# rcedgar/muscle

Hardware: AMD Instinct MI355X
Metric: sequence-pairs/sec (fwd+bwd+posterior+relax) (higher is better)
Workload: dtype f32

## Files before the change

### muscle_amd/csrc/kernels_store.h

```cpp
#pragma once
#include "device_math.h"

struct __attribute__((aligned(8))) MpcEnt { u32 p; u32 c; };

struct StoreParams {
	u32 n;
	const u32 *seq_len;
	u64 npairs;
	const u32 *pair_x, *pair_y;
	u32 *packed;
	const u64 *pbase;
	const u64 *vbase;
	u32 *rp;
	const u64 *rp_base;
	MpcEnt *ent;
	const u64 *ent_base;
	const u32 *mbase;
	float *vnext;
	u32 *pad;
	u32 lcap1;
	unsigned short *pos_f, *pos_t;
	const u32 *rec_off;
	u32 *ovf_off;
	u32 nb1;
	u32 *win;
	const u32 *wrec_off;
	u32 *wv_off;
	unsigned short *pos_wf, *pos_wt;
	u32 nrect;
	const u32 *rects;
	const u8 *need;
	const u64 *pad_zbase, *win_zbase;
	const u32 *pad_zend, *win_zend;
};

#define MPC_PAD_ROW 2
#define MPC_WIN_MAXSPAN 31u
#define MPC_WIN_MAXOFF 32767u
#define MPC_RB_HB 8u
#define MPC_PAD_SENTINEL 0x1fffu

__device__ __forceinline__ u64 mpc_pair_index(u32 n, u32 i, u32 j)
{
	return (u64)i * n - ((u64)i * (i + 1)) / 2 + (j - i - 1);
}

__device__ __forceinline__ u64 mpc_pair_pos_f(u32 n, u32 nrect, const u32 *rects, u32 X, u32 Y)
{
	if (nrect == 0u) return mpc_pair_index(n, X, Y);
	for (u32 r = 0; r < nrect; ++r) {
		const u32 *q = rects + 6u * r;
		const u32 xa = q[0], xb = q[1], ya = q[2], yb = q[3];
		if (X < xa || X >= xb || Y < ya || Y >= yb) continue;
		const u64 base = (u64)q[4] | ((u64)q[5] << 32);
		return ya >= xb ? base + (u64)(X - xa) * (yb - ya) + (Y - ya) : base + mpc_pair_index(xb - xa, X - xa, Y - xa);
	}
	return ~0ull;
}
__device__ __forceinline__ u64 mpc_pair_pos(const StoreParams &s, u32 X, u32 Y) { return mpc_pair_pos_f(s.n, s.nrect, s.rects, X, Y); }
__device__ __forceinline__ bool mpc_need(const StoreParams &s, u32 A) { return s.need == nullptr || s.need[A] != 0; }

__device__ __forceinline__ u64 mpc_rec_index(u32 n, u32 A, u32 Z) { return (u64)Z * n + A; }
__device__ __forceinline__ u32 *mpc_rec_ptr(const StoreParams &s, u32 A, u32 Z)
{
	u32 *base = s.pad_zbase ? (u32 *)s.pad_zbase[Z] : s.pad;
	return base + 4 * (u64)s.rec_off[mpc_rec_index(s.n, A, Z)];
}
__device__ __forceinline__ u32 *mpc_wrec_ptr(const StoreParams &s, u32 A, u32 Z)
{
	u32 *base = s.win_zbase ? (u32 *)s.win_zbase[Z] : s.win;
	return base + 4 * (u64)s.wrec_off[mpc_rec_index(s.n, A, Z)];
}
__device__ __forceinline__ u32 mpc_rec_end(const StoreParams &s, u32 A, u32 Z) { return (s.pad_zend && A + 1u == s.n) ? s.pad_zend[Z] : s.rec_off[mpc_rec_index(s.n, A, Z) + 1]; }
__device__ __forceinline__ u32 mpc_wrec_end(const StoreParams &s, u32 A, u32 Z) { return (s.win_zend && A + 1u == s.n) ? s.win_zend[Z] : s.wrec_off[mpc_rec_index(s.n, A, Z) + 1]; }
__device__ __forceinline__ bool mpc_has_win(const StoreParams &s) { return s.win != nullptr || s.win_zbase != nullptr; }

__global__ void __launch_bounds__(64) slab_build_kernel(StoreParams s)
{
	const int t = threadIdx.x;
	const u64 total = (u64)s.n * s.n;
	for (u64 b = blockIdx.x; b < total; b += gridDim.x) {
		const u32 A = (u32)(b / s.n), Z = (u32)(b % s.n);
		const u32 LA = s.seq_len[A];
		u32 *rp = s.rp + s.rp_base[A] + (u64)Z * (LA + 1);
		const u32 mb = s.mbase[(u64)A * (s.n + 1) + Z];
		if (A == Z) {
			for (u32 a = t; a <= LA; a += 64) rp[a] = mb;
			continue;
		}
		const bool fwd = A < Z;
		const u64 k = fwd ? mpc_pair_pos(s, A, Z) : mpc_pair_pos(s, Z, A);
		const u32 *rec = s.packed + s.pbase[k];
		const u32 LX = fwd ? LA : s.seq_len[Z];
		const u32 LY = fwd ? s.seq_len[Z] : LA;
		const u32 nnz = (u32)(s.vbase[k + 1] - s.vbase[k]);
		const u32 *cnt = fwd ? rec : rec + LX;
		u32 carry = mb;
		for (u32 a0 = 0; a0 <= LA; a0 += 64) {
			const u32 a = a0 + t;
			const u32 v = (a < LA) ? cnt[a] : 0;
			u32 incl = v;
			for (int d = 1; d < 64; d <<= 1) {
				const u32 o = __shfl_up(incl, d);
				if (t >= d) incl += o;
			}
			if (a <= LA) rp[a] = carry + incl - v;
			carry += __shfl(incl, 63);
		}
		const u32 *e = rec + LX + LY;
		const u32 *rowv = e + 2 * (u64)nnz;
		const u32 *tperm = rowv + nnz;
		MpcEnt *dst = s.ent + s.ent_base[A] + mb;
		for (u32 q = t; q < nnz; q += 64) {
			MpcEnt v;
			v.p = e[2 * (u64)q];
			if (fwd) { v.c = e[2 * (u64)q + 1]; dst[q] = v; }
			else { v.c = rowv[q]; dst[tperm[q]] = v; }
		}
	}
}

__global__ void __launch_bounds__(64) var_size_kernel(StoreParams s, u32 *sizes)
{
	const int t = threadIdx.x;
	const u64 total = (u64)s.n * s.n;
	for (u64 b = blockIdx.x; b < total; b += gridDim.x) {
		const u32 Z = (u32)(b / s.n), A = (u32)(b % s.n);
		const u32 LA = s.seq_len[A];
		u32 mine = 0;
		if (!mpc_need(s, A)) { if (t == 0) sizes[b] = 0u; continue; }
		if (A != Z) {
			const bool fwd = A < Z;
			const u64 k = fwd ? mpc_pair_pos(s, A, Z) : mpc_pair_pos(s, Z, A);
			const u32 *rec = s.packed + s.pbase[k];
			const u32 *cnt = fwd ? rec : rec + s.seq_len[Z];
			for (u32 a = t; a < LA; a += 64) {
				const u32 nb = (cnt[a] + MPC_PAD_ROW - 1) / MPC_PAD_ROW;
				mine += nb > 1 ? nb - 1 : 0;
			}
			for (int d = 32; d >= 1; d >>= 1) mine += __shfl_down(mine, d);
		}
		if (t == 0) sizes[b] = LA + mine;
	}
}

__global__ void __launch_bounds__(64) var_build_kernel(StoreParams s)
{
	MPC_DYN_SMEM(smem_raw);
	u32 *s_start = (u32 *)smem_raw;
	u32 *s_ovf = s_start + s.lcap1;
	const int t = threadIdx.x;
	const u64 total = (u64)s.n * s.n;
	for (u64 b = blockIdx.x; b < total; b += gridDim.x) {
		const u32 Z = (u32)(b / s.n), A = (u32)(b % s.n);
		const u32 LA = s.seq_len[A];
		if (!mpc_need(s, A)) continue;
		u32 *rec_out = mpc_rec_ptr(s, A, Z);
		const u32 rec_end = mpc_rec_end(s, A, Z);
		const u32 units = rec_end - s.rec_off[b];
		for (u32 q = t; q < units; q += 64) {
			rec_out[4 * q] = 0u; rec_out[4 * q + 1] = 0u; rec_out[4 * q + 2] = MPC_PAD_SENTINEL; rec_out[4 * q + 3] = MPC_PAD_SENTINEL;
		}
		if (A == Z) {
			if (s.ovf_off) for (u32 q = t; q < s.nb1; q += 64) s.ovf_off[b * s.nb1 + q] = rec_end;
			continue;
		}
		const bool fwd = A < Z;
		const u64 k = fwd ? mpc_pair_pos(s, A, Z) : mpc_pair_pos(s, Z, A);
		const u32 *rec = s.packed + s.pbase[k];
		const u32 LX = fwd ? LA : s.seq_len[Z];
		const u32 LY = fwd ? s.seq_len[Z] : LA;
		const u32 nnz = (u32)(s.vbase[k + 1] - s.vbase[k]);
		const u32 *cnt = fwd ? rec : rec + LX;
		u32 carry = 0, carry_o = 0;
		for (u32 a0 = 0; a0 < LA; a0 += 64) {
			const u32 a = a0 + t;
			const u32 v = (a < LA) ? cnt[a] : 0;
			const u32 nb = (v + MPC_PAD_ROW - 1) / MPC_PAD_ROW;
			const u32 vo = nb > 1 ? nb - 1 : 0;
			u32 incl = v, incl_o = vo;
			for (int d = 1; d < 64; d <<= 1) {
				const u32 o = __shfl_up(incl, d), oo = __shfl_up(incl_o, d);
				if (t >= d) { incl += o; incl_o += oo; }
			}
			if (a < LA) {
				s_start[a] = carry + incl - v;
				s_ovf[a] = carry_o + incl_o - vo;
			}
			carry += __shfl(incl, 63);
			carry_o += __shfl(incl_o, 63);
		}
		__syncthreads();
		if (s.ovf_off)
			for (u32 q = t; q < s.nb1; q += 64)
				s.ovf_off[b * s.nb1 + q] = MPC_RB_HB * q < LA ? s.rec_off[b] + LA + s_ovf[MPC_RB_HB * q] : rec_end;
		const u32 *e = rec + LX + LY;
		const u32 *rowv = e + 2 * (u64)nnz;
		const u32 *tperm = rowv + nnz;
		unsigned short *pos = (fwd ? s.pos_f : s.pos_t) + s.vbase[k];
		for (u32 q = t; q < nnz; q += 64) {
			const u32 pbits = e[2 * (u64)q];
			const u32 col = e[2 * (u64)q + 1], row = rowv[q];
			const u32 r = fwd ? row : col;
			const u32 rank = fwd ? q : tperm[q];
			const u32 c = fwd ? col : row;
			const u32 within = rank - s_start[r];
			const u32 j = within / MPC_PAD_ROW, slot = within % MPC_PAD_ROW;
			const u32 nb = (cnt[r] + MPC_PAD_ROW - 1) / MPC_PAD_ROW;
			const u32 ovf0 = LA + s_ovf[r];
			const u32 unit = j == 0 ? r : ovf0 + (j - 1);
			const u32 delta = j + 1 < nb ? (j == 0 ? ovf0 - r : 1u) : 0u;
			rec_out[4 * unit + slot] = pbits;
			rec_out[4 * unit + 2 + slot] = slot == 0 ? (c | (delta << 20)) : c;
			if (slot == 0 && within + 1 == cnt[r]) rec_out[4 * unit + 3] = c;
			pos[q] = (unsigned short)(unit * MPC_PAD_ROW + slot);
		}
		__syncthreads();
	}
}

__global__ void __launch_bounds__(64) win_size_kernel(StoreParams s, u32 *sizes, u32 *vals_total, u32 *too_wide)
{
	const int t = threadIdx.x;
	const u64 total = (u64)s.n * s.n;
	for (u64 b = blockIdx.x; b < total; b += gridDim.x) {
		const u32 Z = (u32)(b / s.n), A = (u32)(b % s.n);
		const u32 LA = s.seq_len[A];
		u32 mine = 0;
		if (!mpc_need(s, A)) { if (t == 0) { sizes[b] = 0u; vals_total[b] = 0u; } continue; }
		if (A != Z) {
			const u32 *rec = mpc_rec_ptr(s, A, Z);
			for (u32 a = t; a < LA; a += 64) {
				u32 blk = a;
				const u32 c_first = rec[4 * blk + 2] & 0xffffu;
				u32 span = 0;
				if (c_first != MPC_PAD_SENTINEL) {
					for (u32 d = rec[4 * blk + 2] >> 20; d != 0u; d = rec[4 * blk + 2] >> 20) blk += d;
					span = rec[4 * blk + 3] - c_first + 1u;
				}
				mine += span + 1u;
			}
			for (int d = 32; d >= 1; d >>= 1) mine += __shfl_down(mine, d);
		} else mine = LA;
		if (t == 0) {
			sizes[b] = (LA + 1u + 3u) / 4u + (mine + 3u) / 4u + 1u;
			vals_total[b] = mine;
			if (mine > MPC_WIN_MAXOFF) atomicOr(too_wide, 1u);
		}
	}
}

__global__ void __launch_bounds__(64) win_build_kernel(StoreParams s)
{
	MPC_DYN_SMEM(smem_raw);
	u32 *s_off = (u32 *)smem_raw;
	const u32 t = threadIdx.x;
	const u64 total = (u64)s.n * s.n;
	for (u64 b = blockIdx.x; b < total; b += gridDim.x) {
		const u32 Z = (u32)(b / s.n), A = (u32)(b % s.n);
		const u32 LA = s.seq_len[A];
		if (!mpc_need(s, A)) continue;
		const u32 *rec = mpc_rec_ptr(s, A, Z);
		u32 *wrec = mpc_wrec_ptr(s, A, Z);
		const u32 dblocks = (LA + 1u + 3u) / 4u;
		u32 *desc = wrec, *vals = wrec + 4 * (u64)dblocks;
		u32 carry = 0;
		for (u32 a0 = 0; a0 <= LA; a0 += 64) {
			const u32 a = a0 + t;
			u32 c_first = 0, span = 0;
			if (a < LA) {
				u32 blk = a;
				const u32 cf = rec[4 * blk + 2] & 0xffffu;
				if (cf != MPC_PAD_SENTINEL) {
					for (u32 d = rec[4 * blk + 2] >> 20; d != 0u; d = rec[4 * blk + 2] >> 20) blk += d;
					c_first = cf; span = rec[4 * blk + 3] - cf + 1u;
				}
			}
			const u32 v = a < LA ? span + 1u : 0u;
			u32 incl = v;
			for (int d = 1; d < 64; d <<= 1) {
				const u32 o = __shfl_up(incl, d);
				if (t >= (u32)d) incl += o;
			}
			const u32 off = carry + incl - v;
			if (a <= LA) { desc[a] = c_first | ((span < MPC_WIN_MAXSPAN ? span : MPC_WIN_MAXSPAN) << 12) | (off << 17); s_off[a] = off; }
			carry += __shfl(incl, 63);
		}
		for (u32 q = LA + 1u + t; q < 4u * dblocks; q += 64) desc[q] = carry << 17;
		__syncthreads();
		const u32 vtotal = carry, vblocks = (vtotal + 3u) / 4u + 1u;
		for (u32 q = t; q < 4u * vblocks; q += 64) vals[q] = 0u;
		if (s.wv_off)
			for (u32 q = t; q < s.nb1; q += 64)
				s.wv_off[b * s.nb1 + q] = MPC_RB_HB * q < LA ? s.wrec_off[b] + dblocks + s_off[MPC_RB_HB * q] / 4u : mpc_wrec_end(s, A, Z) - 1u;
		__syncthreads();
		for (u32 a = t; a < LA; a += 64) {
			u32 blk = a;
			const u32 cf = rec[4 * blk + 2] & 0xffffu;
			if (cf == MPC_PAD_SENTINEL) continue;
			const u32 off = s_off[a];
			for (;;) {
				const u32 c0 = rec[4 * blk + 2] & 0xffffu, c1 = rec[4 * blk + 3];
				vals[off + (c0 - cf)] = rec[4 * blk];
				if (c1 != c0) vals[off + (c1 - cf)] = rec[4 * blk + 1];
				const u32 d = rec[4 * blk + 2] >> 20;
				if (d == 0u) break;
				blk += d;
			}
		}
		__syncthreads();
	}
}

__global__ void __launch_bounds__(64) win_pos_kernel(StoreParams s)
{
	const u32 t = threadIdx.x;
	for (u64 k = blockIdx.x; k < s.npairs; k += gridDim.x) {
		const u32 X = s.pair_x[k], Y = s.pair_y[k];
		const u32 LX = s.seq_len[X], LY = s.seq_len[Y];
		const u32 *prec = s.packed + s.pbase[k];
		const u32 *ent = prec + LX + LY;
		const u32 nnz = (u32)(s.vbase[k + 1] - s.vbase[k]);
		const bool nx = mpc_need(s, X), ny = mpc_need(s, Y);
		if (!nx && !ny) continue;
		const u32 *dxy = mpc_wrec_ptr(s, X, Y);
		const u32 *dyx = mpc_wrec_ptr(s, Y, X);
		for (u32 q = t; q < nnz; q += 64) {
			const u32 col = ent[2 * (u64)q + 1], row = ent[2 * (u64)nnz + q];
			if (nx) { const u32 wf = dxy[row]; s.pos_wf[s.vbase[k] + q] = (unsigned short)((wf >> 17) + (col - (wf & 0xfffu))); }
			if (ny) { const u32 wt = dyx[col]; s.pos_wt[s.vbase[k] + q] = (unsigned short)((wt >> 17) + (row - (wt & 0xfffu))); }
		}
	}
}

__device__ __forceinline__ void mpc_tile_runs(u32 x0, u32 nx, u32 y0, u32 ny, u32 *ys, u32 *nys)
{
	const u32 lo = y0 > x0 + nx ? y0 : x0 + nx, hi = y0 + ny;
	*ys = lo;
	*nys = hi > lo ? hi - lo : 0u;
}

__global__ void __launch_bounds__(64) var_tile_fit_kernel(StoreParams s, const u32 *tiles, u32 ntiles, u32 *out)
{
	const u32 t = threadIdx.x, n = s.n;
	for (u32 tl = blockIdx.x; tl < ntiles; tl += gridDim.x) {
		const u32 x0 = tiles[4 * tl], nx = tiles[4 * tl + 1], y0 = tiles[4 * tl + 2], ny = tiles[4 * tl + 3];
		u32 ys, nys;
		mpc_tile_runs(x0, nx, y0, ny, &ys, &nys);
		u32 best = 0;
		for (u32 Z = t; Z < n; Z += 64) {
			const u64 bx = mpc_rec_index(n, x0, Z);
			u32 sum = mpc_rec_end(s, x0 + nx - 1u, Z) - s.rec_off[bx];
			if (nys) { const u64 by = mpc_rec_index(n, ys, Z); sum += mpc_rec_end(s, ys + nys - 1u, Z) - s.rec_off[by]; }
			best = sum > best ? sum : best;
		}
		for (int d = 32; d >= 1; d >>= 1) { const u32 o = __shfl_down(best, d); best = o > best ? o : best; }
		if (t == 0) out[tl] = best;
	}
}

__device__ __forceinline__ u64 mpc_find_pair(const u64 *vbase, u64 lo, u64 hi, u64 e)
{
	while (hi - lo > 1) {
		const u64 mid = (lo + hi) >> 1;
		if (vbase[mid] <= e) lo = mid; else hi = mid;
	}
	return lo;
}

__global__ void __launch_bounds__(256) relax_kernel(StoreParams s, u64 k0, u64 k1)
{
	const u64 first = s.vbase[k0], last = s.vbase[k1];
	const u32 n = s.n;
	for (u64 e = first + (u64)blockIdx.x * blockDim.x + threadIdx.x; e < last; e += (u64)gridDim.x * blockDim.x) {
		const u64 k = mpc_find_pair(s.vbase, k0, k1, e);
		const u32 X = s.pair_x[k], Y = s.pair_y[k];
		const u32 LX = s.seq_len[X], LY = s.seq_len[Y];
		const u32 *rec = s.packed + s.pbase[k];
		const u32 nnz = (u32)(s.vbase[k + 1] - s.vbase[k]);
		const u32 idx = (u32)(e - s.vbase[k]);
		const u32 *ent = rec + LX + LY;
		const float pxy = __uint_as_float(ent[2 * (u64)idx]);
		const u32 y = ent[2 * (u64)idx + 1];
		const u32 x = ent[2 * (u64)nnz + idx];
		float acc = pxy * 2.0f;
		const u32 *rpx = s.rp + s.rp_base[X] + x;
		const u32 *rpy = s.rp + s.rp_base[Y] + y;
		const MpcEnt *ex = s.ent + s.ent_base[X];
		const MpcEnt *ey = s.ent + s.ent_base[Y];
		const u32 sxs = LX + 1, sys = LY + 1;
		for (u32 Z = 0; Z < n; ++Z) {
			u32 a = rpx[0], a1 = rpx[1];
			u32 b = rpy[0], b1 = rpy[1];
			rpx += sxs; rpy += sys;
			if (a == a1 || b == b1) continue;
			MpcEnt va = ex[a], vb = ey[b];
			for (;;) {
				if (va.c == vb.c) {
					acc += __uint_as_float(va.p) * __uint_as_float(vb.p);
					if (++a == a1 || ++b == b1) break;
					va = ex[a]; vb = ey[b];
				} else if (va.c < vb.c) {
					if (++a == a1) break;
					va = ex[a];
				} else {
					if (++b == b1) break;
					vb = ey[b];
				}
			}
		}
		s.vnext[e] = acc / (float)n;
	}
}

__global__ void __launch_bounds__(256) commit_kernel(StoreParams s, u64 e0, u64 e1)
{
	const u64 last = e1;
	for (u64 e = e0 + (u64)blockIdx.x * blockDim.x + threadIdx.x; e < last; e += (u64)gridDim.x * blockDim.x) {
		const u64 k = mpc_find_pair(s.vbase, 0, s.npairs, e);
		const u32 X = s.pair_x[k], Y = s.pair_y[k];
		const u32 LX = s.seq_len[X], LY = s.seq_len[Y];
		u32 *rec = s.packed + s.pbase[k];
		const u32 nnz = (u32)(s.vbase[k + 1] - s.vbase[k]);
		const u32 idx = (u32)(e - s.vbase[k]);
		u32 *ent = rec + LX + LY;
		const u32 pb = __float_as_uint(s.vnext[e]);
		const u32 tq = ent[3 * (u64)nnz + idx];
		ent[2 * (u64)idx] = pb;
		s.ent[s.ent_base[X] + s.mbase[(u64)X * (s.n + 1) + Y] + idx].p = pb;
		s.ent[s.ent_base[Y] + s.mbase[(u64)Y * (s.n + 1) + X] + tq].p = pb;
	}
}

__global__ void __launch_bounds__(64) commit_pairs_kernel(StoreParams s, u64 k0, u64 k1, u64 e0, u64 e1, u64 own0, u64 own1, int lazy_packed)
{
	const u32 t = threadIdx.x;
	for (u64 k = k0 + blockIdx.x; k < k1; k += gridDim.x) {
		const u32 X = s.pair_x[k], Y = s.pair_y[k];
		const bool nx = mpc_need(s, X), ny = mpc_need(s, Y);
		const bool pk = !lazy_packed || (k >= own0 && k < own1);
		if (!nx && !ny && !pk) continue;
		const u64 vb = s.vbase[k], ve = s.vbase[k + 1];
		const u64 a = vb > e0 ? vb : e0, b = ve < e1 ? ve : e1;
		if (a >= b) continue;
		const u32 LX = s.seq_len[X], LY = s.seq_len[Y];
		u32 *ent = s.packed + s.pbase[k] + LX + LY;
		u32 *rx = mpc_rec_ptr(s, X, Y), *ry = mpc_rec_ptr(s, Y, X);
		const bool hw = mpc_has_win(s);
		u32 *wx = hw ? mpc_wrec_ptr(s, X, Y) + 4 * (u64)((LX + 1u + 3u) / 4u) : nullptr;
		u32 *wy = hw ? mpc_wrec_ptr(s, Y, X) + 4 * (u64)((LY + 1u + 3u) / 4u) : nullptr;
		for (u64 e = a + t; e < b; e += 64) {
			const u32 pb = __float_as_uint(s.vnext[e]);
			if (pk) ent[2 * (e - vb)] = pb;
			if (nx) { const u32 pf = s.pos_f[e]; rx[(pf >> 1) * 4u + (pf & 1u)] = pb; if (wx) wx[s.pos_wf[e]] = pb; }
			if (ny) { const u32 pt = s.pos_t[e]; ry[(pt >> 1) * 4u + (pt & 1u)] = pb; if (wy) wy[s.pos_wt[e]] = pb; }
		}
	}
}

__global__ void __launch_bounds__(64) packed_refresh_kernel(StoreParams s, u64 k0, u64 k1, u64 e0, u64 e1, u64 own0, u64 own1)
{
	const u32 t = threadIdx.x;
	for (u64 k = k0 + blockIdx.x; k < k1; k += gridDim.x) {
		if (k >= own0 && k < own1) continue;
		const u64 vb = s.vbase[k], ve = s.vbase[k + 1];
		const u64 a = vb > e0 ? vb : e0, b = ve < e1 ? ve : e1;
		u32 *ent = s.packed + s.pbase[k] + s.seq_len[s.pair_x[k]] + s.seq_len[s.pair_y[k]];
		for (u64 e = a + t; e < b; e += 64) ent[2 * (e - vb)] = __float_as_uint(s.vnext[e]);
	}
}

__global__ void __launch_bounds__(256) pack_kernel(const u32 *res, u64 res_stride, const u64 *dst_base,
	const u64 *rec_words, u32 *packed, u32 count)
{
	for (u32 pid = blockIdx.x; pid < count; pid += gridDim.x) {
		const u32 *src = res + (u64)pid * res_stride;
		u32 *dst = packed + dst_base[pid];
		const u64 w = rec_words[pid];
		for (u64 q = threadIdx.x; q < w; q += blockDim.x) dst[q] = src[q];
	}
}

__global__ void __launch_bounds__(64) export_kernel(StoreParams s, u64 k0, u64 k1, const u64 *off_base,
	u32 *out_off, u32 *out_val, const u64 *klist, const u64 *val_base)
{
	const int t = threadIdx.x;
	for (u64 q = k0 + blockIdx.x; q < k1; q += gridDim.x) {
		const u64 k = klist ? klist[q] : q;
		const u32 LX = s.seq_len[s.pair_x[k]], LY = s.seq_len[s.pair_y[k]];
		const u32 *rec = s.packed + s.pbase[k];
		const u32 nnz = (u32)(s.vbase[k + 1] - s.vbase[k]);
		u32 *oo = out_off + off_base[q - k0];
		u32 carry = 0;
		for (u32 a0 = 0; a0 <= LX; a0 += 64) {
			const u32 a = a0 + t;
			const u32 v = (a < LX) ? rec[a] : 0;
			u32 incl = v;
			for (int d = 1; d < 64; d <<= 1) {
				const u32 o = __shfl_up(incl, d);
				if (t >= d) incl += o;
			}
			if (a <= LX) oo[a] = carry + incl - v;
			carry += __shfl(incl, 63);
		}
		const u32 *ent = rec + LX + LY;
		u32 *ov = out_val + 2 * (klist ? val_base[q] : s.vbase[k] - s.vbase[k0]);
		for (u32 i = t; i < 2 * nnz; i += 64) ov[i] = ent[i];
	}
}
```

### muscle_amd/csrc/mpcgpu_store.inc

```

const u64 kStoreSegBlocksMax = 0xffffffffull;

bool plan_store_segments(u32 n, const u32 *sizes, u64 limit, std::vector<u32> &z_first, std::vector<u64> &blocks)
{
	z_first.assign(1, 0u);
	blocks.assign(1, 0ull);
	for (u32 Z = 0; Z < n; ++Z) {
		u64 slab = 0;
		for (u32 A = 0; A < n; ++A) slab += sizes[(u64)Z * n + A];
		if (slab > limit) return false;
		if (blocks.back() + slab > limit) { z_first.push_back(Z); blocks.push_back(0ull); }
		blocks.back() += slab;
	}
	return true;
}

u64 store_seg_limit()
{
	const char *e = getenv("MPCGPU_STORE_SEG_BLOCKS");
	const u64 v = (e && *e) ? strtoull(e, nullptr, 10) : 0ull;
	return (v == 0ull || v > kStoreSegBlocksMax) ? kStoreSegBlocksMax : v;
}

void segment_offsets(u32 n, std::vector<u32> &off, const std::vector<u32> &z_first, std::vector<u32> &zend)
{
	zend.resize(n);
	u64 run = 0;
	size_t g = 0;
	for (u32 Z = 0; Z < n; ++Z) {
		if (g + 1 < z_first.size() && Z == z_first[g + 1]) { ++g; run = 0; }
		for (u32 A = 0; A < n; ++A) {
			const u64 b = (u64)Z * n + A;
			const u32 sz = off[b + 1];
			off[b] = (u32)run;
			run += sz;
		}
		zend[Z] = (u32)run;
	}
	off[(u64)n * n] = (u32)run;
}

bool segments_held(const DevBuf &one, const SegStore &st, const std::vector<u64> &blocks)
{
	if (blocks.size() == 1) return one.cap >= std::max<u64>(blocks[0], 1) * 16;
	if (st.seg.size() != blocks.size()) return false;
	for (size_t g = 0; g < blocks.size(); ++g)
		if (st.seg[g].cap < std::max<u64>(blocks[g], 1) * 16) return false;
	return true;
}

int alloc_segments(mpcgpu_ctx *c, SegStore &st, const std::vector<u32> &z_first, const std::vector<u64> &blocks, const std::vector<u32> &zend)
{
	const u32 n = c->n;
	for (size_t g = blocks.size(); g < st.seg.size(); ++g) st.seg[g].release();
	st.seg.resize(blocks.size());
	std::vector<u64> zb(n);
	for (size_t g = 0; g < blocks.size(); ++g) {
		HIPCHK(c, st.seg[g].ensure(std::max<u64>(blocks[g], 1) * 16));
		const u32 z1 = g + 1 < blocks.size() ? z_first[g + 1] : n;
		for (u32 Z = z_first[g]; Z < z1; ++Z) zb[Z] = (u64)(uintptr_t)st.seg[g].p;
	}
	if (upload(c, st.zbase, zb) || upload(c, st.zend, zend)) return 1;
	HIPCHK(c, hipStreamSynchronize(c->stream));
	return 0;
}

int build_var_store(mpcgpu_ctx *c)
{
	const u32 n = c->n;
	if (c->max_len > MPC_RV_MAXLEN) return 2;
	StoreParams sp0;
	fill_store_params(c, sp0);
	const u64 nn = (u64)n * n;
	HIPCHK(c, c->d_sizes.ensure(nn * 4));
	MPC_LAUNCH(var_size_kernel, (u32)std::min<u64>(nn, (u64)c->prop.multiProcessorCount * 32), 64, 0, c->stream, sp0, c->d_sizes.as<u32>());
	HIPCHK(c, hipGetLastError());
	std::vector<u32> &off = c->v_off;
	off.resize(nn + 1);
	HIPCHK(c, hipMemcpyAsync(off.data() + 1, c->d_sizes.p, nn * 4, hipMemcpyDeviceToHost, c->stream));
	HIPCHK(c, hipStreamSynchronize(c->stream));
	off[0] = 0;
	u32 max_rec = 0;
	u64 run = 0;
	for (u64 b = 0; b < nn; ++b) { max_rec = std::max(max_rec, off[b + 1]); run += off[b + 1]; }
	if (max_rec > 4095u) return 2;
	const u64 seg_limit = store_seg_limit();
	std::vector<u32> seg_z, zend;
	std::vector<u64> seg_blocks;
	if (!plan_store_segments(n, off.data() + 1, seg_limit, seg_z, seg_blocks)) return 2;
	const u32 nseg = (u32)seg_blocks.size();
	segment_offsets(n, off, seg_z, zend);
	auto fits = [&](bool fallback) {
		return 2ull * max_rec * 16 <= var_buf_bytes(fallback) && (((u64)c->max_nnz + 63) & ~63ull) <= (u64)var_max_slots(fallback) * 1024u;
	};
	const bool fits_primary = fits(false), pairs_ok = fits_primary || fits(true);
	const char *tiles_mode = getenv("MPCGPU_RELAX_TILES");
	const int small_n = env_int("MPCGPU_RELAX_SMALL_PAIRS", 0);
	const bool small_pairs = small_n > 0 && n <= (u32)small_n && fits_primary && !(tiles_mode && !strcmp(tiles_mode, "band")) && nseg == 1;
	const bool want_band = !(tiles_mode && !strcmp(tiles_mode, "pairs")) && !small_pairs && c->npairs < 0xffffffffull;
	if (nseg > 1 && tiles_mode && !strcmp(tiles_mode, "pairs"))
		return fail(c, "MPCGPU_RELAX_TILES=pairs: the whole-record tiles of relax_var_kernel do not read a record store in segments "
			"(%u segments of at most %llu blocks; band tiles do)", nseg, (u64)seg_limit);
	c->var_mixed = !fits_primary && pairs_ok;
	if (!pairs_ok && !want_band) return 2;
	if (nseg > 1 && !want_band) return 2;
	const u64 pad_bytes = run * 16 + 4 * std::max<u64>(c->total_entries, 1);
	const bool held = segments_held(c->d_pad, c->pad_seg, seg_blocks) && 4 * std::max<u64>(c->total_entries, 1) <= c->d_pos.cap;
	if (!segments_held(c->d_pad, c->pad_seg, seg_blocks)) { c->d_pad.release(); c->pad_seg.release(); }
	size_t freeb = 0, totb = 0;
	HIPCHK(c, hipMemGetInfo(&freeb, &totb));
	if (!(held || pad_bytes + ((u64)2 << 30) <= (u64)freeb)) return 2;
	c->d_rp.release(); c->d_ent.release(); c->d_mbase.release();
	if (nseg == 1) {
		c->pad_seg.release();
		HIPCHK(c, c->d_pad.ensure(std::max<u64>(run, 1) * 16));
	} else {
		c->d_pad.release();
		if (alloc_segments(c, c->pad_seg, seg_z, seg_blocks, zend)) return 1;
	}
	HIPCHK(c, c->d_pos.ensure(4 * std::max<u64>(c->total_entries, 1)));
	if (upload(c, c->d_rec_off, off)) return 1;
	HIPCHK(c, hipStreamSynchronize(c->stream));
	c->have_pad = true;
	c->pad_lcap1 = c->max_len;
	c->var_max_rec_blocks = max_rec; c->var_total_blocks = run;
	c->tiles_k0 = c->tiles_k1 = ~0ull;
	{
		char b[512];
		snprintf(b, sizeof(b), "variable-size dense records: %u x %u records, %.2f GB, mean %.0f B, largest %u B; relax_var_kernel, 2 x 1024-thread workgroups per CU, 1 staging buffer of %u B",
			n, n, (double)run * 16 / 1e9, (double)run * 16 / (double)nn, max_rec * 16, var_buf_bytes(false));
		c->store_desc = b;
		if (c->var_mixed) c->store_desc += " (pairs whose records do not fit it: 1 x 1024-thread workgroup per CU with 160 KB, second launch)";
		if (nseg > 1) c->store_desc += " in " + std::to_string(nseg) + " segments of whole Z slabs";
		c->tiles_desc.clear(); c->relax_kernel_name.clear(); c->relax_fallback = false;
	}
	c->band_ok = false;
	c->btiles_k0 = c->btiles_k1 = ~0ull;
	{
		const u32 nb1 = (c->max_len + MPC_RB_HB - 1) / MPC_RB_HB + 1;
		const u64 tab_bytes = (nn + 2 * c->npairs + 2ull * n) * nb1 * 4;
		size_t free2 = 0, tot2 = 0;
		HIPCHK(c, hipMemGetInfo(&free2, &tot2));
		if (want_band && (c->d_ovf_off.cap >= nn * nb1 * 4 || tab_bytes + ((u64)1 << 30) <= (u64)free2)) {
			HIPCHK(c, c->d_ovf_off.ensure(nn * nb1 * 4));
			HIPCHK(c, c->d_cell_off.ensure(std::max<u64>(c->npairs, 1) * nb1 * 4));
			HIPCHK(c, c->d_yr.ensure(std::max<u64>(c->npairs, 1) * nb1 * 4));
			HIPCHK(c, c->d_ovf_sum.ensure(3ull * n * nb1 * 4));
			HIPCHK(c, c->d_ovf_maxc.ensure((u64)n * nb1 * 4));
			c->band_ok = true;
			c->band_nb1 = nb1;
			char b[256];
			snprintf(b, sizeof(b), "variable-size dense records: %u x %u records, %.2f GB, mean %.0f B, largest %u B, band index of %u rows",
				n, n, (double)run * 16 / 1e9, (double)run * 16 / (double)nn, max_rec * 16, (unsigned)MPC_RB_HB);
			c->store_desc = b;
			if (nseg > 1) c->store_desc += ", in " + std::to_string(nseg) + " segments of whole Z slabs";
		}
		if (!c->band_ok && (!pairs_ok || nseg > 1)) { c->have_pad = false; return 2; }
		c->var_pairs_ok = pairs_ok && nseg == 1;
	}
	StoreParams sp;
	fill_store_params(c, sp);
	if (trace_on()) {
		fprintf(stderr, "[mpcgpu] store: variable-size dense records, %u x %u records, %.2f GB (mean %.0f B, largest %u B)%s\n", n, n,
			(double)run * 16 / 1e9, (double)run * 16 / (double)nn, max_rec * 16, c->var_mixed ? ", relax_var fallback for the largest pairs" : "");
		fflush(stderr);
	}
	TimedSpan ts;
	if (span_begin(c, 2, &ts)) return 1;
	MPC_LAUNCH(var_build_kernel, (u32)std::min<u64>(nn, (u64)c->prop.multiProcessorCount * 32), 64, (size_t)std::max(sp.lcap1, 1u) * 8, c->stream, sp);
	HIPCHK(c, hipGetLastError());
	c->win_ok = false;
	{
		const char *form = getenv("MPCGPU_RELAX_FORM");
		if (c->band_ok && !(form && !strcmp(form, "walk"))) {
			HIPCHK(c, c->d_sizes.ensure(nn * 4));
			HIPCHK(c, c->d_tilefit.ensure(nn * 4));
			HIPCHK(c, c->d_wflag.ensure(4));
			HIPCHK(c, hipMemsetAsync(c->d_wflag.p, 0, 4, c->stream));
			MPC_LAUNCH(win_size_kernel, (u32)std::min<u64>(nn, (u64)c->prop.multiProcessorCount * 32), 64, 0, c->stream, sp, c->d_sizes.as<u32>(),
				c->d_tilefit.as<u32>(), c->d_wflag.as<u32>());
			HIPCHK(c, hipGetLastError());
			std::vector<u32> &woff = c->v_woff;
			woff.resize(nn + 1);
			u32 wide = 0;
			HIPCHK(c, hipMemcpyAsync(woff.data() + 1, c->d_sizes.p, nn * 4, hipMemcpyDeviceToHost, c->stream));
			HIPCHK(c, hipMemcpyAsync(&wide, c->d_wflag.p, 4, hipMemcpyDeviceToHost, c->stream));
			HIPCHK(c, hipStreamSynchronize(c->stream));
			woff[0] = 0;
			u64 wrun = 0;
			for (u64 b = 0; b < nn; ++b) wrun += woff[b + 1];
			std::vector<u32> wseg_z, wzend;
			std::vector<u64> wseg_blocks;
			const bool wplan = plan_store_segments(n, woff.data() + 1, seg_limit, wseg_z, wseg_blocks);
			const u32 nwseg = wplan ? (u32)wseg_blocks.size() : 0u;
			if (wplan) segment_offsets(n, woff, wseg_z, wzend);
			const double ratio = (double)wrun / (double)std::max<u64>(run, 1);
			const double max_ratio = (double)env_int("MPCGPU_RELAX_WIN_PCT", 125) / 100.0;
			const bool wheld = wplan && segments_held(c->d_win, c->win_seg, wseg_blocks);
			if (!wheld) { c->d_win.release(); c->win_seg.release(); }
			size_t free3 = 0, tot3 = 0;
			HIPCHK(c, hipMemGetInfo(&free3, &tot3));
			const u64 need = wrun * 16 + 4 * std::max<u64>(c->total_entries, 1) + nn * c->band_nb1 * 4;
			if (!wide && wplan && ratio <= max_ratio && (wheld || need + ((u64)1 << 30) <= (u64)free3)) {
				if (nwseg == 1) {
					c->win_seg.release();
					HIPCHK(c, c->d_win.ensure(std::max<u64>(wrun, 1) * 16));
				} else {
					c->d_win.release();
					if (alloc_segments(c, c->win_seg, wseg_z, wseg_blocks, wzend)) return 1;
				}
				HIPCHK(c, c->d_pos_w.ensure(4 * std::max<u64>(c->total_entries, 1)));
				HIPCHK(c, c->d_wv_off.ensure(nn * c->band_nb1 * 4));
				HIPCHK(c, c->d_wsum.ensure(3ull * n * c->band_nb1 * 4));
				HIPCHK(c, c->d_wmaxc.ensure((u64)n * c->band_nb1 * 4));
				if (upload(c, c->d_wrec_off, woff)) return 1;
				HIPCHK(c, hipStreamSynchronize(c->stream));
				c->win_ok = true;
				c->win_total_blocks = wrun;
				fill_store_params(c, sp);
				MPC_LAUNCH(win_build_kernel, (u32)std::min<u64>(nn, (u64)c->prop.multiProcessorCount * 32), 64, (size_t)(std::max(sp.lcap1, 1u) + 1) * 4, c->stream, sp);
				HIPCHK(c, hipGetLastError());
				MPC_LAUNCH(win_pos_kernel, (u32)std::min<u64>(std::max<u64>(c->npairs, 1), (u64)c->prop.multiProcessorCount * 32), 64, 0, c->stream, sp);
				HIPCHK(c, hipGetLastError());
				MPC_LAUNCH(ovf_stats_kernel, std::min<u32>(n, (u32)c->prop.multiProcessorCount * 32), 64, 0, c->stream, sp, c->d_wv_off.as<u32>(), c->band_nb1,
					c->d_wsum.as<u32>(), c->d_wmaxc.as<u32>(), 1);
				HIPCHK(c, hipGetLastError());
				char wb[160];
				snprintf(wb, sizeof(wb), " + window records for the Y operand (%.2f GB, %.0f %% of the blocks)", (double)wrun * 16 / 1e9, 100.0 * ratio);
				c->store_desc += wb;
				if (nwseg > 1) c->store_desc += " in " + std::to_string(nwseg) + " segments";
			} else {
				if (trace_on())
					fprintf(stderr, "[mpcgpu] store: no window records (%s; they would take %.0f %% of the block records' %.2f GB)\n",
						wide ? "a record's windows exceed 65535 values" : !wplan ? "one Z slab of them passes the segment limit" : ratio > max_ratio ? "rows too wide" : "device memory",
						100.0 * ratio, (double)run * 16 / 1e9);
			}
		}
	}
	if (!c->win_ok) release_windows(c);
	if (c->band_ok) {
		MPC_LAUNCH(band_index_kernel, (u32)std::min<u64>(std::max<u64>(c->npairs, 1), (u64)c->prop.multiProcessorCount * 32), 64, 0, c->stream, sp, c->band_nb1,
			c->d_cell_off.as<u32>(), c->d_yr.as<u32>());
		HIPCHK(c, hipGetLastError());
		MPC_LAUNCH(ovf_stats_kernel, std::min<u32>(n, (u32)c->prop.multiProcessorCount * 32), 64, 0, c->stream, sp, c->d_ovf_off.as<u32>(), c->band_nb1,
			c->d_ovf_sum.as<u32>(), c->d_ovf_maxc.as<u32>(), 0);
		HIPCHK(c, hipGetLastError());
	}
	if (span_end(c, &ts)) return 1;
	HIPCHK(c, hipStreamSynchronize(c->stream));
	return 0;
}
```

Baseline: 344,500.

## Fuse record and window sizing and building into single-pass kernels

```diff
diff --git a/muscle_amd/csrc/kernels_store.h b/muscle_amd/csrc/kernels_store.h
--- a/muscle_amd/csrc/kernels_store.h
+++ b/muscle_amd/csrc/kernels_store.h
@@ -330,6 +330,171 @@
 			if (nx) { const u32 wf = dxy[row]; s.pos_wf[s.vbase[k] + q] = (unsigned short)((wf >> 17) + (col - (wf & 0xfffu))); }
 			if (ny) { const u32 wt = dyx[col]; s.pos_wt[s.vbase[k] + q] = (unsigned short)((wt >> 17) + (row - (wt & 0xfffu))); }
 		}
+	}
+}
+
+__global__ void __launch_bounds__(64) rec_size_kernel(StoreParams s, u32 *sizes, u32 *wsizes, u32 *too_wide, int want_win)
+{
+	MPC_DYN_SMEM(smem_raw);
+	u32 *s_hi = (u32 *)smem_raw;
+	u32 *s_lo = s_hi + s.lcap1;
+	const u32 t = threadIdx.x;
+	const u64 total = (u64)s.n * s.n;
+	for (u64 b = blockIdx.x; b < total; b += gridDim.x) {
+		const u32 Z = (u32)(b / s.n), A = (u32)(b % s.n);
+		const u32 LA = s.seq_len[A];
+		if (!mpc_need(s, A)) { if (t == 0) { sizes[b] = 0u; if (want_win) wsizes[b] = 0u; } continue; }
+		u32 ovf = 0, vals = LA;
+		if (A != Z) {
+			const bool fwd = A < Z;
+			const u64 k = fwd ? mpc_pair_pos(s, A, Z) : mpc_pair_pos(s, Z, A);
+			const u32 *rec = s.packed + s.pbase[k];
+			const u32 LX = fwd ? LA : s.seq_len[Z], LY = fwd ? s.seq_len[Z] : LA;
+			const u32 *cnt = fwd ? rec : rec + LX;
+			for (u32 a = t; a < LA; a += 64) {
+				const u32 nb = (cnt[a] + MPC_PAD_ROW - 1) / MPC_PAD_ROW;
+				ovf += nb > 1 ? nb - 1 : 0;
+				if (want_win) { s_hi[a] = 0u; s_lo[a] = 0u; }
+			}
+			if (want_win) {
+				const u32 nnz = (u32)(s.vbase[k + 1] - s.vbase[k]);
+				const u32 *e = rec + LX + LY;
+				const u32 *rowv = e + 2 * (u64)nnz;
+				__syncthreads();
+				for (u32 q = t; q < nnz; q += 64) {
+					const u32 col = e[2 * (u64)q + 1], row = rowv[q];
+					const u32 r = fwd ? row : col, c = fwd ? col : row;
+					atomicMax(&s_hi[r], c + 1u);
+					atomicMax(&s_lo[r], 0x10000u - c);
+				}
+				__syncthreads();
+				vals = 0;
+				for (u32 a = t; a < LA; a += 64) {
+					const u32 hi = s_hi[a];
+					vals += (hi ? hi - (0x10000u - s_lo[a]) : 0u) + 1u;
+				}
+				__syncthreads();
+			}
+			for (int d = 32; d >= 1; d >>= 1) { ovf += __shfl_down(ovf, d); vals += __shfl_down(vals, d); }
+		}
+		if (t == 0) {
+			sizes[b] = LA + ovf;
+			if (want_win) {
+				wsizes[b] = (LA + 1u + 3u) / 4u + (vals + 3u) / 4u + 1u;
+				if (vals > MPC_WIN_MAXOFF) atomicOr(too_wide, 1u);
+			}
+		}
+	}
+}
+
+template <bool WIN>
+__global__ void __launch_bounds__(64) rec_build_kernel(StoreParams s)
+{
+	MPC_DYN_SMEM(smem_raw);
+	u32 *s_so = (u32 *)smem_raw;
+	u32 *s_off = s_so + s.lcap1;
+	unsigned short *s_fl = (unsigned short *)(s_off + s.lcap1 + 1);
+	const u32 t = threadIdx.x;
+	const u64 total = (u64)s.n * s.n;
+	for (u64 b = blockIdx.x; b < total; b += gridDim.x) {
+		const u32 Z = (u32)(b / s.n), A = (u32)(b % s.n);
+		const u32 LA = s.seq_len[A];
+		if (!mpc_need(s, A)) continue;
+		u32 *rec_out = mpc_rec_ptr(s, A, Z);
+		const u32 rec_end = mpc_rec_end(s, A, Z);
+		const u32 units = rec_end - s.rec_off[b];
+		for (u32 q = t; q < units; q += 64) {
+			rec_out[4 * q] = 0u; rec_out[4 * q + 1] = 0u; rec_out[4 * q + 2] = MPC_PAD_SENTINEL; rec_out[4 * q + 3] = MPC_PAD_SENTINEL;
+		}
+		const bool fwd = A < Z, diag = A == Z;
+		const u64 k = diag ? 0ull : fwd ? mpc_pair_pos(s, A, Z) : mpc_pair_pos(s, Z, A);
+		const u32 *rec = s.packed + (diag ? 0ull : s.pbase[k]);
+		const u32 LX = fwd ? LA : s.seq_len[Z];
+		const u32 LY = fwd ? s.seq_len[Z] : LA;
+		const u32 nnz = diag ? 0u : (u32)(s.vbase[k + 1] - s.vbase[k]);
+		const u32 *cnt = fwd ? rec : rec + LX;
+		u32 carry = 0, carry_o = 0;
+		for (u32 a0 = 0; a0 < LA; a0 += 64) {
+			const u32 a = a0 + t;
+			const u32 v = (a < LA && !diag) ? cnt[a] : 0;
+			const u32 nb = (v + MPC_PAD_ROW - 1) / MPC_PAD_ROW;
+			const u32 vo = nb > 1 ? nb - 1 : 0;
+			u32 incl = v, incl_o = vo;
+			for (int d = 1; d < 64; d <<= 1) {
+				const u32 o = __shfl_up(incl, d), oo = __shfl_up(incl_o, d);
+				if (t >= (u32)d) { incl += o; incl_o += oo; }
+			}
+			if (a < LA) s_so[a] = (carry + incl - v) | ((carry_o + incl_o - vo) << 16);
+			carry += __shfl(incl, 63);
+			carry_o += __shfl(incl_o, 63);
+		}
+		__syncthreads();
+		if (s.ovf_off)
+			for (u32 q = t; q < s.nb1; q += 64)
+				s.ovf_off[b * s.nb1 + q] = MPC_RB_HB * q < LA ? s.rec_off[b] + LA + (s_so[MPC_RB_HB * q] >> 16) : rec_end;
+		const u32 *e = rec + LX + LY;
+		const u32 *rowv = e + 2 * (u64)nnz;
+		const u32 *tperm = rowv + nnz;
+		unsigned short *pos = (fwd ? s.pos_f : s.pos_t) + (diag ? 0ull : s.vbase[k]);
+		for (u32 q = t; q < nnz; q += 64) {
+			const u32 pbits = e[2 * (u64)q];
+			const u32 col = e[2 * (u64)q + 1], row = rowv[q];
+			const u32 r = fwd ? row : col;
+			const u32 rank = fwd ? q : tperm[q];
+			const u32 c = fwd ? col : row;
+			const u32 so = s_so[r], cr = cnt[r];
+			const u32 within = rank - (so & 0xffffu);
+			const u32 j = within / MPC_PAD_ROW, slot = within % MPC_PAD_ROW;
+			const u32 nb = (cr + MPC_PAD_ROW - 1) / MPC_PAD_ROW;
+			const u32 ovf0 = LA + (so >> 16);
+			const u32 unit = j == 0 ? r : ovf0 + (j - 1);
+			const u32 delta = j + 1 < nb ? (j == 0 ? ovf0 - r : 1u) : 0u;
+			rec_out[4 * unit + slot] = pbits;
+			rec_out[4 * unit + 2 + slot] = slot == 0 ? (c | (delta << 20)) : c;
+			if (slot == 0 && within + 1 == cr) rec_out[4 * unit + 3] = c;
+			pos[q] = (unsigned short)(unit * MPC_PAD_ROW + slot);
+			if (WIN) {
+				if (within == 0u) s_fl[2 * r] = (unsigned short)c;
+				if (within + 1u == cr) s_fl[2 * r + 1] = (unsigned short)c;
+			}
+		}
+		if (WIN) {
+			u32 *wrec = mpc_wrec_ptr(s, A, Z);
+			const u32 dblocks = (LA + 1u + 3u) / 4u;
+			u32 *desc = wrec, *vals = wrec + 4 * (u64)dblocks;
+			__syncthreads();
+			u32 wcarry = 0;
+			for (u32 a0 = 0; a0 <= LA; a0 += 64) {
+				const u32 a = a0 + t;
+				u32 c_first = 0, span = 0;
+				if (a < LA && !diag && cnt[a] != 0u) { c_first = s_fl[2 * a]; span = s_fl[2 * a + 1] - c_first + 1u; }
+				const u32 v = a < LA ? span + 1u : 0u;
+				u32 incl = v;
+				for (int d = 1; d < 64; d <<= 1) {
+					const u32 o = __shfl_up(incl, d);
+					if (t >= (u32)d) incl += o;
+				}
+				const u32 off = wcarry + incl - v;
+				if (a <= LA) { desc[a] = c_first | ((span < MPC_WIN_MAXSPAN ? span : MPC_WIN_MAXSPAN) << 12) | (off << 17); s_off[a] = off; }
+				wcarry += __shfl(incl, 63);
+			}
+			for (u32 q = LA + 1u + t; q < 4u * dblocks; q += 64) desc[q] = wcarry << 17;
+			const u32 vblocks = (wcarry + 3u) / 4u + 1u;
+			for (u32 q = t; q < 4u * vblocks; q += 64) vals[q] = 0u;
+			__syncthreads();
+			if (s.wv_off)
+				for (u32 q = t; q < s.nb1; q += 64)
+					s.wv_off[b * s.nb1 + q] = MPC_RB_HB * q < LA ? s.wrec_off[b] + dblocks + s_off[MPC_RB_HB * q] / 4u : mpc_wrec_end(s, A, Z) - 1u;
+			unsigned short *posw = (fwd ? s.pos_wf : s.pos_wt) + (diag ? 0ull : s.vbase[k]);
+			for (u32 q = t; q < nnz; q += 64) {
+				const u32 col = e[2 * (u64)q + 1], row = rowv[q];
+				const u32 r = fwd ? row : col, c = fwd ? col : row;
+				const u32 w = s_off[r] + (c - s_fl[2 * r]);
+				vals[w] = e[2 * (u64)q];
+				posw[q] = (unsigned short)w;
+			}
+		}
+		__syncthreads();
 	}
 }
 
diff --git a/muscle_amd/csrc/mpcgpu_store.inc b/muscle_amd/csrc/mpcgpu_store.inc
--- a/muscle_amd/csrc/mpcgpu_store.inc
+++ b/muscle_amd/csrc/mpcgpu_store.inc
@@ -69,15 +69,38 @@
 {
 	const u32 n = c->n;
 	if (c->max_len > MPC_RV_MAXLEN) return 2;
+	const char *build_mode = getenv("MPCGPU_STORE_BUILD");
+	const bool passes = build_mode && !strcmp(build_mode, "passes");
+	const char *form = getenv("MPCGPU_RELAX_FORM");
+	const char *tiles_mode = getenv("MPCGPU_RELAX_TILES");
 	StoreParams sp0;
 	fill_store_params(c, sp0);
+	sp0.lcap1 = c->max_len;
 	const u64 nn = (u64)n * n;
-	HIPCHK(c, c->d_sizes.ensure(nn * 4));
-	MPC_LAUNCH(var_size_kernel, (u32)std::min<u64>(nn, (u64)c->prop.multiProcessorCount * 32), 64, 0, c->stream, sp0, c->d_sizes.as<u32>());
-	HIPCHK(c, hipGetLastError());
-	std::vector<u32> &off = c->v_off;
+	const u32 rec_grid = (u32)std::min<u64>(nn, (u64)c->prop.multiProcessorCount * 32);
+	std::vector<u32> &off = c->v_off, &woff = c->v_woff;
 	off.resize(nn + 1);
-	HIPCHK(c, hipMemcpyAsync(off.data() + 1, c->d_sizes.p, nn * 4, hipMemcpyDeviceToHost, c->stream));
+	const bool size_win = !passes && !(form && !strcmp(form, "walk")) && !(tiles_mode && !strcmp(tiles_mode, "pairs")) && c->npairs < 0xffffffffull;
+	u32 wide = 0;
+	if (passes) {
+		HIPCHK(c, c->d_sizes.ensure(nn * 4));
+		MPC_LAUNCH(var_size_kernel, rec_grid, 64, 0, c->stream, sp0, c->d_sizes.as<u32>());
+		HIPCHK(c, hipGetLastError());
+		HIPCHK(c, hipMemcpyAsync(off.data() + 1, c->d_sizes.p, nn * 4, hipMemcpyDeviceToHost, c->stream));
+	} else {
+		HIPCHK(c, c->d_sizes.ensure((2 * nn + 1) * 4));
+		u32 *d_flag = c->d_sizes.as<u32>() + 2 * nn;
+		HIPCHK(c, hipMemsetAsync(d_flag, 0, 4, c->stream));
+		MPC_LAUNCH(rec_size_kernel, rec_grid, 64, size_win ? (size_t)std::max(sp0.lcap1, 1u) * 8 : 0, c->stream, sp0, c->d_sizes.as<u32>(),
+			c->d_sizes.as<u32>() + nn, d_flag, size_win ? 1 : 0);
+		HIPCHK(c, hipGetLastError());
+		HIPCHK(c, hipMemcpyAsync(off.data() + 1, c->d_sizes.p, nn * 4, hipMemcpyDeviceToHost, c->stream));
+		if (size_win) {
+			woff.resize(nn + 1);
+			HIPCHK(c, hipMemcpyAsync(woff.data() + 1, c->d_sizes.as<u32>() + nn, nn * 4, hipMemcpyDeviceToHost, c->stream));
+			HIPCHK(c, hipMemcpyAsync(&wide, d_flag, 4, hipMemcpyDeviceToHost, c->stream));
+		}
+	}
 	HIPCHK(c, hipStreamSynchronize(c->stream));
 	off[0] = 0;
 	u32 max_rec = 0;
@@ -94,7 +117,6 @@
 		return 2ull * max_rec * 16 <= var_buf_bytes(fallback) && (((u64)c->max_nnz + 63) & ~63ull) <= (u64)var_max_slots(fallback) * 1024u;
 	};
 	const bool fits_primary = fits(false), pairs_ok = fits_primary || fits(true);
-	const char *tiles_mode = getenv("MPCGPU_RELAX_TILES");
 	const int small_n = env_int("MPCGPU_RELAX_SMALL_PAIRS", 0);
 	const bool small_pairs = small_n > 0 && n <= (u32)small_n && fits_primary && !(tiles_mode && !strcmp(tiles_mode, "band")) && nseg == 1;
 	const bool want_band = !(tiles_mode && !strcmp(tiles_mode, "pairs")) && !small_pairs && c->npairs < 0xffffffffull;
@@ -120,7 +142,7 @@
 	}
 	HIPCHK(c, c->d_pos.ensure(4 * std::max<u64>(c->total_entries, 1)));
 	if (upload(c, c->d_rec_off, off)) return 1;
-	HIPCHK(c, hipStreamSynchronize(c->stream));
+	if (passes) HIPCHK(c, hipStreamSynchronize(c->stream));
 	c->have_pad = true;
 	c->pad_lcap1 = c->max_len;
 	c->var_max_rec_blocks = max_rec; c->var_total_blocks = run;
@@ -167,25 +189,25 @@
 	}
 	TimedSpan ts;
 	if (span_begin(c, 2, &ts)) return 1;
-	MPC_LAUNCH(var_build_kernel, (u32)std::min<u64>(nn, (u64)c->prop.multiProcessorCount * 32), 64, (size_t)std::max(sp.lcap1, 1u) * 8, c->stream, sp);
-	HIPCHK(c, hipGetLastError());
+	if (passes) {
+		MPC_LAUNCH(var_build_kernel, rec_grid, 64, (size_t)std::max(sp.lcap1, 1u) * 8, c->stream, sp);
+		HIPCHK(c, hipGetLastError());
+	}
 	c->win_ok = false;
 	{
-		const char *form = getenv("MPCGPU_RELAX_FORM");
 		if (c->band_ok && !(form && !strcmp(form, "walk"))) {
-			HIPCHK(c, c->d_sizes.ensure(nn * 4));
-			HIPCHK(c, c->d_tilefit.ensure(nn * 4));
-			HIPCHK(c, c->d_wflag.ensure(4));
-			HIPCHK(c, hipMemsetAsync(c->d_wflag.p, 0, 4, c->stream));
-			MPC_LAUNCH(win_size_kernel, (u32)std::min<u64>(nn, (u64)c->prop.multiProcessorCount * 32), 64, 0, c->stream, sp, c->d_sizes.as<u32>(),
-				c->d_tilefit.as<u32>(), c->d_wflag.as<u32>());
-			HIPCHK(c, hipGetLastError());
-			std::vector<u32> &woff = c->v_woff;
-			woff.resize(nn + 1);
-			u32 wide = 0;
-			HIPCHK(c, hipMemcpyAsync(woff.data() + 1, c->d_sizes.p, nn * 4, hipMemcpyDeviceToHost, c->stream));
-			HIPCHK(c, hipMemcpyAsync(&wide, c->d_wflag.p, 4, hipMemcpyDeviceToHost, c->stream));
-			HIPCHK(c, hipStreamSynchronize(c->stream));
+			if (passes) {
+				HIPCHK(c, c->d_sizes.ensure(nn * 4));
+				HIPCHK(c, c->d_tilefit.ensure(nn * 4));
+				HIPCHK(c, c->d_wflag.ensure(4));
+				HIPCHK(c, hipMemsetAsync(c->d_wflag.p, 0, 4, c->stream));
+				MPC_LAUNCH(win_size_kernel, rec_grid, 64, 0, c->stream, sp, c->d_sizes.as<u32>(), c->d_tilefit.as<u32>(), c->d_wflag.as<u32>());
+				HIPCHK(c, hipGetLastError());
+				woff.resize(nn + 1);
+				HIPCHK(c, hipMemcpyAsync(woff.data() + 1, c->d_sizes.p, nn * 4, hipMemcpyDeviceToHost, c->stream));
+				HIPCHK(c, hipMemcpyAsync(&wide, c->d_wflag.p, 4, hipMemcpyDeviceToHost, c->stream));
+				HIPCHK(c, hipStreamSynchronize(c->stream));
+			}
 			woff[0] = 0;
 			u64 wrun = 0;
 			for (u64 b = 0; b < nn; ++b) wrun += woff[b + 1];
@@ -218,10 +240,16 @@
 				c->win_ok = true;
 				c->win_total_blocks = wrun;
 				fill_store_params(c, sp);
-				MPC_LAUNCH(win_build_kernel, (u32)std::min<u64>(nn, (u64)c->prop.multiProcessorCount * 32), 64, (size_t)(std::max(sp.lcap1, 1u) + 1) * 4, c->stream, sp);
-				HIPCHK(c, hipGetLastError());
-				MPC_LAUNCH(win_pos_kernel, (u32)std::min<u64>(std::max<u64>(c->npairs, 1), (u64)c->prop.multiProcessorCount * 32), 64, 0, c->stream, sp);
-				HIPCHK(c, hipGetLastError());
+				if (passes) {
+					MPC_LAUNCH(win_build_kernel, rec_grid, 64, (size_t)(std::max(sp.lcap1, 1u) + 1) * 4, c->stream, sp);
+					HIPCHK(c, hipGetLastError());
+					MPC_LAUNCH(win_pos_kernel, (u32)std::min<u64>(std::max<u64>(c->npairs, 1), (u64)c->prop.multiProcessorCount * 32), 64, 0, c->stream, sp);
+					HIPCHK(c, hipGetLastError());
+				} else {
+					const size_t smem = ((size_t)std::max(sp.lcap1, 1u) * 3 + 1) * 4;
+					MPC_LAUNCH(rec_build_kernel<true>, rec_grid, 64, smem, c->stream, sp);
+					HIPCHK(c, hipGetLastError());
+				}
 				MPC_LAUNCH(ovf_stats_kernel, std::min<u32>(n, (u32)c->prop.multiProcessorCount * 32), 64, 0, c->stream, sp, c->d_wv_off.as<u32>(), c->band_nb1,
 					c->d_wsum.as<u32>(), c->d_wmaxc.as<u32>(), 1);
 				HIPCHK(c, hipGetLastError());
@@ -237,6 +265,11 @@
 			}
 		}
 	}
+	if (!passes && !c->win_ok) {
+		HIPCHK(c, hipStreamSynchronize(c->stream));
+		MPC_LAUNCH(rec_build_kernel<false>, rec_grid, 64, (size_t)std::max(sp.lcap1, 1u) * 4, c->stream, sp);
+		HIPCHK(c, hipGetLastError());
+	}
 	if (!c->win_ok) release_windows(c);
 	if (c->band_ok) {
 		MPC_LAUNCH(band_index_kernel, (u32)std::min<u64>(std::max<u64>(c->npairs, 1), (u64)c->prop.multiProcessorCount * 32), 64, 0, c->stream, sp, c->band_nb1,
```

Result: no change. 346,300 (median of 6 runs) (+0.5%).
